# deryrahman/image-caption-emotion-indonesia

Measured on AMD Instinct MI355X. Metric: images/sec (train step) + NLL loss match, batch=64 ResNet152+FactoredLSTM-512, higher is better.
Workload: dtype f32 (trunk: operands as 2 f16 pieces each, 3 MFMA products per multiply, f32 accumulate; decoder: large products as 3 bf16 pieces per operand, 6 MFMA products per multiply, the rest f32 MFMA; the persistent LSTM kernel the trunk's split-f16 scheme)

## Files before the change

### image-caption-emotion-indonesia_amd/csrc/fused_block.hip

```cpp
#include <cstdlib>
#include <type_traits>

#include "common.h"
#include "mfma_core.h"
#include "kernels.h"

namespace capnet {
namespace {

typedef _Float16 h8 __attribute__((ext_vector_type(8)));
typedef _Float16 h4 __attribute__((ext_vector_type(4)));
typedef _Float16 h2 __attribute__((ext_vector_type(2)));
typedef float f2 __attribute__((ext_vector_type(2)));

constexpr int kFHdr = 4;

__host__ __device__ constexpr int fb_kslot(int g, int j) { return 16 * (j >> 2) + 4 * g + (j & 3); }

__device__ __forceinline__ void fb_split4(const f32x4 v, h4& h, h4& l) {
  const f2 a = {v[0], v[1]}, b = {v[2], v[3]};
  const h2 ha = __builtin_convertvector(a, h2), hb = __builtin_convertvector(b, h2);
  const f2 ra = a - __builtin_convertvector(ha, f2), rb = b - __builtin_convertvector(hb, f2);
  const h2 la = __builtin_convertvector(ra, h2), lb = __builtin_convertvector(rb, h2);
  h = h4{ha[0], ha[1], hb[0], hb[1]};
// ... 242 lines not shown
}

constexpr int kQC = 16;

template <int K>
__global__ __launch_bounds__(K * 4) void fb_quad_kernel(const float* __restrict__ G, const float* __restrict__ mu,
                                                        const float* __restrict__ w , int C, double inv_count,
                                                        double unbias, const float* __restrict__ gamma, const float* __restrict__ beta,
                                                        float* __restrict__ running_mean, float* __restrict__ running_var,
                                                        float momentum, float eps, float* __restrict__ scale, float* __restrict__ shift,
                                                        float* __restrict__ batch_mean, float* __restrict__ batch_var, int* __restrict__ err) {
  constexpr int NW = K / 16, S = K / 4, SB = S < 32 ? S : 32;
  __shared__ float red[2][kQC][NW];
  const int tid = threadIdx.x, lane = tid & 63, nb = tid >> 6, g4 = lane >> 4, ln = lane & 15, c0 = blockIdx.x * kQC;
  const float* wq = w + (long)blockIdx.x * K * kQC;
  f32x4 acc = {0.f, 0.f, 0.f, 0.f};
#pragma unroll
  for (int s0 = 0; s0 < S; s0 += SB) {
    float a[SB], b[SB];
#pragma unroll
    for (int i = 0; i < SB; ++i) {
      const int k = 4 * (s0 + i) + g4;
      a[i] = wq[k * kQC + ln];
      b[i] = G[(long)k * K + 16 * nb + ln];
    }
#pragma unroll
    for (int i = 0; i < SB; ++i) acc = __builtin_amdgcn_mfma_f32_16x16x4f32(a[i], b[i], acc, 0, 0, 0);
  }
  const int col = 16 * nb + ln;
  const f32x4 wv = *reinterpret_cast<const f32x4*>(wq + col * kQC + 4 * g4);
  const float m = mu[col];
#pragma unroll
  for (int r = 0; r < 4; ++r) {
    float q = acc[r] * wv[r], sm = m * wv[r];
#pragma unroll
    for (int o = 1; o < 16; o <<= 1) {
      q += __shfl_xor(q, o);
      sm += __shfl_xor(sm, o);
    }
    if (ln == 0) { red[0][4 * g4 + r][nb] = q; red[1][4 * g4 + r][nb] = sm; }
  }
  __syncthreads();
  if (tid < kQC && c0 + tid < C) {
    const int c = c0 + tid;
    double qq = 0.0, ss = 0.0;
#pragma unroll
    for (int v = 0; v < NW; ++v) { qq += (double)red[0][tid][v]; ss += (double)red[1][tid][v]; }
    if (err && !(qq < __builtin_inf())) atomicOr(err, 8);
    const double mean = ss * inv_count;
    double var = qq * inv_count - mean * mean;
    if (var < 0.0) var = 0.0;
    const float invstd = (float)(1.0 / sqrt(var + (double)eps));
    const float gm = gamma ? gamma[c] : 1.f, bt = beta ? beta[c] : 0.f;
    const float sc = gm * invstd;
    scale[c] = sc;
    shift[c] = bt - (float)mean * sc;
    if (running_mean) {
      running_mean[c] = __builtin_fmaf(momentum, (float)mean, (1.f - momentum) * running_mean[c]);
      running_var[c] = __builtin_fmaf(momentum, (float)(var * unbias), (1.f - momentum) * running_var[c]);
    }
    if (batch_mean) {
      batch_mean[c] = (float)mean;
      batch_var[c] = (float)(var * unbias);
    }
  }
}

struct FArgs {
  const float* y2; const float* s2; const float* t2;
  const unsigned* w3; const unsigned* w1;
  const float* s3; const float* t3;
  const float* res; const float* sd; const float* td;
  float* out; float* y1; float* part_sum; float* part_sq;
  int M, e3, e1;
  int* err;
};

#ifndef CAPNET_FB_DBG
#define CAPNET_FB_DBG 0
#endif
template <int N>
__device__ __forceinline__ void fb_wait_vmcnt() { asm volatile("s_waitcnt vmcnt(%0)" ::"n"(N) : "memory"); }

template <int MID, int RS, int NW>
__global__ __launch_bounds__(64 * NW, NW / 4) void fb_fused_kernel(const FArgs g) {
  constexpr int C = 4 * MID, KS = MID / 32, NB = MID / 16, NCH = C / 32;
  constexpr int SLOT = MID * 128;
  constexpr int NDMA = SLOT / 1024 / NW;
  constexpr int L = 2 * RS;
  constexpr int TR = 16 * RS * NW;
  constexpr int NT = 64 * NW;
  static_assert(NDMA >= 1 && 4 * NDMA + 2 * L <= 63, "vmcnt range");
  __shared__ __attribute__((aligned(16))) unsigned char ring[4 * SLOT];
  __shared__ __attribute__((aligned(16))) float par[4][C];
  const int tid = threadIdx.x, lane = tid & 63, wave = tid >> 6, gq = lane >> 4, ln = lane & 15;
  const int wave_u = __builtin_amdgcn_readfirstlane(wave);
  const unsigned ring0 = __builtin_amdgcn_readfirstlane((unsigned)(size_t)(__attribute__((address_space(3))) unsigned char*)ring);
  const int tile0 = (int)blockIdx.x * TR;
  const bool fold_res = g.sd != nullptr;
  const float* const w3img = reinterpret_cast<const float*>(g.w3 + kFHdr);
  const float* const w1img = reinterpret_cast<const float*>(g.w1 + kFHdr);

  auto dma = [&](const float* img, int cc, int slot) __attribute__((always_inline)) {
    const float* src = img + (long)cc * (SLOT / 4);
#pragma unroll
    for (int q = 0; q < ((CAPNET_FB_DBG == 2 || CAPNET_FB_DBG == 4) ? 0 : NDMA); ++q)
      glds16(src, (wave_u * NDMA + q) * 1024 + lane * 16, ring0 + (unsigned)(slot * SLOT + (wave_u * NDMA + q) * 1024));
  };
  unsigned idoff[RS];
#pragma unroll
  for (int s = 0; s < RS; ++s) {
    const int row = min(tile0 + (wave * RS + s) * 16 + ln, g.M - 1);
    idoff[s] = (unsigned)(((long)row * C + 4 * gq) * 4);
  }
  f32x4 idA[RS][2], idB[RS][2];
  auto fetch_id = [&](int cc, f32x4 (&id)[RS][2]) __attribute__((always_inline)) {
#pragma unroll
    for (int s = 0; s < RS; ++s)
#pragma unroll
      for (int blk = 0; blk < 2; ++blk) gload16(id[s][blk], g.res, idoff[s] + (unsigned)((32 * cc + 16 * blk) * 4));
  };

  dma(w3img, 0, 0);
  dma(w1img, 0, 1);
  fetch_id(0, idA);
  fetch_id(NCH > 1 ? 1 : 0, idB);
  {
    const float x3 = ldexpf(1.f, -((int)g.w3[0] + g.e3));
    for (int i = tid; i < C; i += NT) {
      par[0][i] = g.s3[i] * x3;
      par[1][i] = g.t3[i];
      par[2][i] = fold_res ? g.sd[i] : 1.f;
      par[3][i] = fold_res ? g.td[i] : 0.f;
    }
  }
  h8 ah[RS][KS], al[RS][KS];
  {
    const float is3 = ldexpf(1.f, g.e3);
#pragma unroll
    for (int s = 0; s < RS; ++s) {
      const int row = min(tile0 + (wave * RS + s) * 16 + ln, g.M - 1);
      const float* p = g.y2 + (long)row * MID + 4 * gq;
#pragma unroll
      for (int ks = 0; ks < KS; ++ks) {
        f32x4 v0 = *reinterpret_cast<const f32x4*>(p + 32 * ks), v1 = *reinterpret_cast<const f32x4*>(p + 32 * ks + 16);
        const f32x4 sa = *reinterpret_cast<const f32x4*>(g.s2 + 32 * ks + 4 * gq), sb = *reinterpret_cast<const f32x4*>(g.s2 + 32 * ks + 16 + 4 * gq);
        const f32x4 ta = *reinterpret_cast<const f32x4*>(g.t2 + 32 * ks + 4 * gq), tb = *reinterpret_cast<const f32x4*>(g.t2 + 32 * ks + 16 + 4 * gq);
#pragma unroll
        for (int e = 0; e < 4; ++e) {
          v0[e] = fmaxf(fmaf(v0[e], sa[e], ta[e]), 0.f) * is3;
          v1[e] = fmaxf(fmaf(v1[e], sb[e], tb[e]), 0.f) * is3;
        }
        h4 h0, l0, h1, l1;
        fb_split4(v0, h0, l0);
        fb_split4(v1, h1, l1);
        ah[s][ks] = fb_cat(h0, h1);
        al[s][ks] = fb_cat(l0, l1);
      }
    }
  }
  fb_wait_vmcnt<0>();
  CAPNET_LANDED4(idA[0][0], idA[0][1], idB[0][0], idB[0][1]);
  if constexpr (RS == 2) CAPNET_LANDED4(idA[1][0], idA[1][1], idB[1][0], idB[1][1]);
  __syncthreads();

  f32x4 acc[RS][NB];
#pragma unroll
  for (int s = 0; s < RS; ++s)
// ... 74 lines not shown
    for (int bb = 0; bb < FD; ++bb)
      if (bb < NBATB) read_b(bb);
    __builtin_amdgcn_sched_barrier(0);
    fb_wait_vmcnt<4 * NDMA + 2 * L>();
    if constexpr (RS == 2) CAPNET_LANDED4(id[0][0], id[0][1], id[1][0], id[1][1]);
    else CAPNET_LANDED2(id[0][0], id[0][1]);
    h8 oh[RS], ol[RS];
#pragma unroll
    for (int s = 0; s < RS; ++s) {
      const int row = min(tile0 + (wave * RS + s) * 16 + ln, g.M - 1);
      h4 hh[2], ll[2];
#pragma unroll
      for (int blk = 0; blk < 2; ++blk) {
        const int ch = 32 * cc + 16 * blk + 4 * gq;
        const f32x4 sv = *reinterpret_cast<const f32x4*>(&par[0][ch]), tv = *reinterpret_cast<const f32x4*>(&par[1][ch]);
        f32x4 r = id[s][blk], o;
        if (fold_res) {
          const f32x4 dv = *reinterpret_cast<const f32x4*>(&par[2][ch]), ev = *reinterpret_cast<const f32x4*>(&par[3][ch]);
#pragma unroll
          for (int e = 0; e < 4; ++e) r[e] = fmaf(r[e], dv[e], ev[e]);
        }
#pragma unroll
        for (int e = 0; e < 4; ++e) o[e] = fmaxf(fmaf(d[s][blk][e], sv[e], tv[e]) + r[e], 0.f);
        *reinterpret_cast<f32x4*>(g.out + (long)row * C + ch) = o;
        fb_split4(o * is1, hh[blk], ll[blk]);
      }
      oh[s] = fb_cat(hh[0], hh[1]);
      ol[s] = fb_cat(ll[0], ll[1]);
    }
    fetch_id(cc + 2 < NCH ? cc + 2 : NCH - 1, id);
#pragma unroll
    for (int b = 0; b < NBATB; ++b) {
      if (b + FD < NBATB) read_b(b + FD);
      __builtin_amdgcn_sched_barrier(0);
#pragma unroll
      for (int q = 0; q < GB; ++q) {
        const int nb = b * GB + q;
        if (nb < NB) {
#pragma unroll
          for (int s = 0; s < RS; ++s) {
            if (CAPNET_FB_DBG >= 3) continue;
            if (CAPNET_FB_DBG == 1) { asm volatile("" :: "v"(fb[b % (FD + 1)][q][1]), "v"(fb[b % (FD + 1)][q][0])); continue; }
            acc[s][nb] = __builtin_amdgcn_mfma_f32_16x16x32_f16(ol[s], fb[b % (FD + 1)][q][0], acc[s][nb], 0, 0, 0);
            acc[s][nb] = __builtin_amdgcn_mfma_f32_16x16x32_f16(oh[s], fb[b % (FD + 1)][q][1], acc[s][nb], 0, 0, 0);
            acc[s][nb] = __builtin_amdgcn_mfma_f32_16x16x32_f16(oh[s], fb[b % (FD + 1)][q][0], acc[s][nb], 0, 0, 0);
          }
        }
      }
      __builtin_amdgcn_sched_barrier(0);
    }
  };
  auto head = [&](int k) __attribute__((always_inline)) {
    if (k < 4) fb_wait_vmcnt<0>(); else fb_wait_vmcnt<NDMA + 2 * L>();
    __syncthreads();
    const int p = k + 2 < 2 * NCH ? k + 2 : 2 * NCH - 2 + (k & 1);
    dma((p & 1) ? w1img : w3img, p >> 1, (k + 2) & 3);
  };
  static_assert(NCH % 2 == 0, "chunks come in pairs (two named register sets)");
  auto run = [&](auto lag_c) __attribute__((always_inline)) {
    constexpr int LAG = decltype(lag_c)::value;
    for (int k = 0; k < 2 * NCH; k += 4) {
      const int c0 = k >> 1;
      head(k);
      if constexpr (LAG == 0) phase_a(c0);
      else { if (c0 > 0) phase_b(c0 - 1, idB); }
      head(k + 1);
      if constexpr (LAG == 0) phase_b(c0, idA);
      else phase_a(c0);
      head(k + 2);
      if constexpr (LAG == 0) phase_a(c0 + 1);
      else phase_b(c0, idA);
      head(k + 3);
      if constexpr (LAG == 0) phase_b(c0 + 1, idB);
      else phase_a(c0 + 1);
    }
    if constexpr (NW == 8) {
      head(2 * NCH);
      if constexpr (LAG != 0) phase_b(NCH - 1, idB);
    }
    fb_wait_vmcnt<0>();
    CAPNET_LANDED4(idA[0][0], idA[0][1], idB[0][0], idB[0][1]);
    if constexpr (RS == 2) CAPNET_LANDED4(idA[1][0], idA[1][1], idB[1][0], idB[1][1]);
  };
  if (NW == 4 || wave_u < 4) run(std::integral_constant<int, 0>{});
  else run(std::integral_constant<int, 1>{});
  __syncthreads();

  const float osc = ldexpf(1.f, -((int)g.w1[0] + g.e1));
  float (*const scratch)[NW][MID] = reinterpret_cast<float (*)[NW][MID]>(ring);
  float bad = 0.f;
#pragma unroll
  for (int nb = 0; nb < NB; ++nb) {
    float cs = 0.f, cq = 0.f;
#pragma unroll
    for (int s = 0; s < RS; ++s)
#pragma unroll
      for (int i = 0; i < 4; ++i) {
        const int row = tile0 + (wave * RS + s) * 16 + 4 * gq + i;
        const float v = acc[s][nb][i] * osc;
        if (row < g.M) {
          g.y1[(long)row * MID + 16 * nb + ln] = v;
          cs += v;
          cq = fmaf(v, v, cq);
        }
      }
    if (g.part_sum) {
      cs += __shfl_xor(cs, 16); cq += __shfl_xor(cq, 16);
      cs += __shfl_xor(cs, 32); cq += __shfl_xor(cq, 32);
      if (gq == 0) { scratch[0][wave][16 * nb + ln] = cs; scratch[1][wave][16 * nb + ln] = cq; }
    } else {
      bad += cq;
    }
  }
  if (!g.part_sum) {
    if (g.err) flag_nonfinite(bad, g.err);
    return;
  }
  __syncthreads();
  for (int c = tid; c < MID; c += NT) {
    float a = 0.f, b = 0.f;
#pragma unroll
    for (int w = 0; w < NW; ++w) { a += scratch[0][w][c]; b += scratch[1][w][c]; }
    g.part_sum[(long)blockIdx.x * MID + c] = a;
    g.part_sq[(long)blockIdx.x * MID + c] = b;
  }
}

template <int MID>
__global__ __launch_bounds__(256, 1) void fb_fused_wide_kernel(const FArgs g) {
  constexpr int C = 4 * MID, KS = MID / 16, NB = MID / 32, NCH = C / 32, NW = 4;
  constexpr int SLOT = MID * 128;
  constexpr int NDMA = SLOT / 1024 / NW;
  constexpr int L = 4;
  constexpr int TR = 32 * NW;
  constexpr int NT = 64 * NW;
  static_assert(NDMA >= 1 && 4 * NDMA + 2 * L <= 63, "vmcnt range");
  __shared__ __attribute__((aligned(16))) unsigned char ring[4 * SLOT];
  __shared__ __attribute__((aligned(16))) float par[4][C];
  const int tid = threadIdx.x, lane = tid & 63, wave = tid >> 6, lh = lane >> 5, li = lane & 31;
  const int wave_u = __builtin_amdgcn_readfirstlane(wave);
  const unsigned ring0 = __builtin_amdgcn_readfirstlane((unsigned)(size_t)(__attribute__((address_space(3))) unsigned char*)ring);
  const int tile0 = (int)blockIdx.x * TR;
  const bool fold_res = g.sd != nullptr;
  const float* const w3img = reinterpret_cast<const float*>(g.w3 + kFHdr);
  const float* const w1img = reinterpret_cast<const float*>(g.w1 + kFHdr);
  auto dma = [&](const float* img, int cc, int slot) __attribute__((always_inline)) {
    const float* src = img + (long)cc * (SLOT / 4);
#pragma unroll
    for (int q = 0; q < ((CAPNET_FB_DBG == 2 || CAPNET_FB_DBG == 4) ? 0 : NDMA); ++q)
      glds16(src, (wave_u * NDMA + q) * 1024 + lane * 16, ring0 + (unsigned)(slot * SLOT + (wave_u * NDMA + q) * 1024));
  };
  const int myrow = min(tile0 + wave * 32 + li, g.M - 1);
  const unsigned idoff = (unsigned)(((long)myrow * C + 4 * lh) * 4);
  f32x4 idA[4], idB[4];
  auto fetch_id = [&](int cc, f32x4 (&id)[4]) __attribute__((always_inline)) {
#pragma unroll
    for (int q = 0; q < 4; ++q) gload16(id[q], g.res, idoff + (unsigned)((32 * cc + 8 * q) * 4));
  };
  dma(w3img, 0, 0);
  dma(w1img, 0, 1);
  fetch_id(0, idA);
  fetch_id(NCH > 1 ? 1 : 0, idB);
  {
    const float x3 = ldexpf(1.f, -((int)g.w3[0] + g.e3));
    for (int i = tid; i < C; i += NT) {
      par[0][i] = g.s3[i] * x3;
      par[1][i] = g.t3[i];
// ... 179 lines not shown
#pragma unroll
    for (int w = 0; w < NW; ++w) { a += scratch[0][w][c]; b += scratch[1][w][c]; }
    g.part_sum[(long)blockIdx.x * MID + c] = a;
    g.part_sq[(long)blockIdx.x * MID + c] = b;
  }
}

}

bool fused_block_shape_ok(long M, int MID) {
  return (MID == 64 || MID == 128 || MID == 256) && M > 0 && M < (1l << 24) && M * 4 * MID * 4 < (1l << 32);
}

size_t fused_block_weight_words(int C, int MID, int role) {
  return (size_t)kFHdr + (size_t)C * MID * (role == 0 ? 2 : 1);
}

static bool fb_wide(int MID) {
  const char* e = getenv("CAPNET_FB_WIDE");
  if (e && (e[0] == '0' || e[0] == '1')) return e[0] == '1';
  (void)MID;
  return false;
}

int fused_block_pack(const float* w, unsigned* img, int C, int MID, int role, hipStream_t stream) {
  CAPNET_REQUIRE(w && img && aligned16(img) && C == 4 * MID && (MID == 64 || MID == 128 || MID == 256) && (role == 0 || role == 1),
                 "fused_block_pack: bad argument (C=%d MID=%d role=%d)", C, MID, role);
  CAPNET_HIP_CHECK(hipMemsetAsync(img, 0, kFHdr * 4, stream));
  const long n = (long)C * MID;
  hipLaunchKernelGGL(fb_absmax_kernel, dim3((int)(cdiv(n, 256 * 8) > 1024 ? 1024 : cdiv(n, 256 * 8))), dim3(256), 0, stream, w, img, n);
  CAPNET_LAUNCH_CHECK();
  hipLaunchKernelGGL(fb_pack_kernel, dim3((int)(cdiv(n / 4, 256) > 2048 ? 2048 : cdiv(n / 4, 256))), dim3(256), 0, stream, w, img, C, MID, role, fb_wide(MID) ? 1 : 0);
  CAPNET_LAUNCH_CHECK();
  return kOk;
}

int fused_block_gram_slices(long M, int K) { return cdiv(M, fb_gram_rows(K)); }
int fused_block_gram_pairs(int K) { const int nb = K / 64; return nb * (nb + 1) / 2; }
size_t fused_block_stats_floats(long M, int K) {
  const size_t s = fused_block_gram_slices(M, K), p = fused_block_gram_pairs(K);
  return s * p * 4096 + ((s * K + 3) / 4 * 4) + ((size_t)K * K + K) + 8;
}

int fused_block_stats(const float* y2, const float* s2, const float* t2, const unsigned* w3img, long M, int MID, int in_exp,
                      const float* gamma, const float* beta, float* running_mean, float* running_var, float momentum, float eps,
                      float* scale, float* shift, float* batch_mean, float* batch_var, float* work, int* err, hipStream_t stream) {
  CAPNET_REQUIRE(y2 && s2 && t2 && w3img && scale && shift && work && aligned16(work) && aligned16(y2) && fused_block_shape_ok(M, MID) &&
                     in_exp > -64 && in_exp < 64, "fused_block_stats: bad argument");
  const int K = MID, C = 4 * MID;
  GArgs a;
  a.y2 = y2; a.s2 = s2; a.t2 = t2; a.M = (int)M; a.K = K; a.in_exp = in_exp;
  a.slices = fused_block_gram_slices(M, K); a.pairs = fused_block_gram_pairs(K); a.slice_rows = fb_gram_rows(K);
  a.gp = work;
  a.cs = work + (size_t)a.slices * a.pairs * 4096;
  float* G = a.cs + ((size_t)a.slices * K + 3) / 4 * 4;
  float* mu = G + (size_t)K * K;
  if (K == 256) hipLaunchKernelGGL(fb_gram_kernel<256>, dim3(a.slices), dim3(256), 0, stream, a);
  else if (K == 128) hipLaunchKernelGGL(fb_gram_kernel<128>, dim3(a.slices), dim3(256), 0, stream, a);
  else hipLaunchKernelGGL(fb_gram_kernel<64>, dim3(a.slices), dim3(256), 0, stream, a);
  hipLaunchKernelGGL(fb_gram_reduce_kernel, dim3(cdiv((long)K * K + K, 32)), dim3(256), 0, stream, a.gp, a.cs, G, mu, K, a.slices, a.pairs);
  const double inv = 1.0 / (double)M, unbias = M > 1 ? (double)M / (double)(M - 1) : 1.0;
  const float* wcopy = reinterpret_cast<const float*>(w3img + kFHdr + (size_t)C * MID);
  if (K == 256)
    hipLaunchKernelGGL(fb_quad_kernel<256>, dim3(cdiv(C, kQC)), dim3(K * 4), 0, stream, G, mu, wcopy, C, inv, unbias, gamma, beta,
                       running_mean, running_var, momentum, eps, scale, shift, batch_mean, batch_var, err);
  else if (K == 128)
    hipLaunchKernelGGL(fb_quad_kernel<128>, dim3(cdiv(C, kQC)), dim3(K * 4), 0, stream, G, mu, wcopy, C, inv, unbias, gamma, beta,
                       running_mean, running_var, momentum, eps, scale, shift, batch_mean, batch_var, err);
  else
    hipLaunchKernelGGL(fb_quad_kernel<64>, dim3(cdiv(C, kQC)), dim3(K * 4), 0, stream, G, mu, wcopy, C, inv, unbias, gamma, beta,
                       running_mean, running_var, momentum, eps, scale, shift, batch_mean, batch_var, err);
  CAPNET_LAUNCH_CHECK();
  return kOk;
}

static void fb_shape(int MID, int* rs, int* nw) {
  (void)MID;
  const char* e = getenv("CAPNET_FB_RS");
  const char* w = getenv("CAPNET_FB_NW");
  *nw = (w && w[0] == '4') ? 4 : 8;
  *rs = (e && (e[0] == '1' || e[0] == '2')) ? e[0] - '0' : (*nw == 8 ? 1 : 2);
  if (*nw == 8) *rs = 1;
}
int fused_block_tiles(long M, int MID) {
  if (fb_wide(MID)) return cdiv(M, 128);
  int rs, nw;
  fb_shape(MID, &rs, &nw);
  return cdiv(M, 16 * rs * nw);
}

int fused_block_forward(const float* y2, const float* s2, const float* t2, const unsigned* w3img, const float* s3, const float* t3,
                        const float* res, const float* sd, const float* td, float* out, const unsigned* w1img, float* y1,
                        float* part_sum, float* part_sq, long M, int MID, int e3, int e1, int* err, hipStream_t stream) {
  CAPNET_REQUIRE(y2 && s2 && t2 && w3img && s3 && t3 && res && out && w1img && y1 && fused_block_shape_ok(M, MID),
                 "fused_block_forward: bad argument");
  CAPNET_REQUIRE(aligned16(y2) && aligned16(s2) && aligned16(t2) && aligned16(w3img) && aligned16(w1img) && aligned16(res) &&
                     aligned16(out) && (sd == nullptr) == (td == nullptr) && (part_sum == nullptr) == (part_sq == nullptr) &&
                     e3 > -64 && e3 < 64 && e1 > -64 && e1 < 64, "fused_block_forward: alignment / pairs / exponents");
  FArgs a;
  a.y2 = y2; a.s2 = s2; a.t2 = t2; a.w3 = w3img; a.w1 = w1img; a.s3 = s3; a.t3 = t3; a.res = res; a.sd = sd; a.td = td;
  a.out = out; a.y1 = y1; a.part_sum = part_sum; a.part_sq = part_sq; a.M = (int)M; a.e3 = e3; a.e1 = e1; a.err = err;
  const dim3 grid(fused_block_tiles(M, MID));
  int rs, nw;
  fb_shape(MID, &rs, &nw);
  if (fb_wide(MID)) {
    const dim3 block(256);
    if (MID == 256) CAPNET_LAUNCH_TIMED((fb_fused_wide_kernel<256>), grid, block, stream, a);
    else if (MID == 128) CAPNET_LAUNCH_TIMED((fb_fused_wide_kernel<128>), grid, block, stream, a);
    else CAPNET_LAUNCH_TIMED((fb_fused_wide_kernel<64>), grid, block, stream, a);
    CAPNET_LAUNCH_CHECK();
    return kOk;
  }
  const dim3 block(64 * nw);
  if (nw == 8) {
    if (MID == 256) CAPNET_LAUNCH_TIMED((fb_fused_kernel<256, 1, 8>), grid, block, stream, a);
    else if (MID == 128) CAPNET_LAUNCH_TIMED((fb_fused_kernel<128, 1, 8>), grid, block, stream, a);
    else CAPNET_LAUNCH_TIMED((fb_fused_kernel<64, 1, 8>), grid, block, stream, a);
  } else if (rs == 2) {
    if (MID == 256) CAPNET_LAUNCH_TIMED((fb_fused_kernel<256, 2, 4>), grid, block, stream, a);
    else if (MID == 128) CAPNET_LAUNCH_TIMED((fb_fused_kernel<128, 2, 4>), grid, block, stream, a);
    else CAPNET_LAUNCH_TIMED((fb_fused_kernel<64, 2, 4>), grid, block, stream, a);
  } else {
    if (MID == 256) CAPNET_LAUNCH_TIMED((fb_fused_kernel<256, 1, 4>), grid, block, stream, a);
    else if (MID == 128) CAPNET_LAUNCH_TIMED((fb_fused_kernel<128, 1, 4>), grid, block, stream, a);
    else CAPNET_LAUNCH_TIMED((fb_fused_kernel<64, 1, 4>), grid, block, stream, a);
  }
  CAPNET_LAUNCH_CHECK();
  return kOk;
}

}
```

### image-caption-emotion-indonesia_amd/csrc/conv3x3_patch.hip

```cpp
#include <cstdlib>

#include "common.h"
#include "mfma_core.h"
#include "kernels.h"

namespace capnet {
namespace {

typedef _Float16 h8 __attribute__((ext_vector_type(8)));
typedef _Float16 h4 __attribute__((ext_vector_type(4)));
typedef _Float16 h2 __attribute__((ext_vector_type(2)));
typedef float f2 __attribute__((ext_vector_type(2)));
typedef unsigned u4 __attribute__((ext_vector_type(4)));

constexpr int PBM = 128;
constexpr int kPmax = 248;
constexpr int kPatchSub = kPmax * 16;
constexpr int kPatch = 8 * kPatchSub;
constexpr int kThreads = 512;
constexpr int kPL = (kPmax * 8 + kThreads - 1) / kThreads;
constexpr int kHdrWords = 4;
static_assert(kPmax % 16 == 8 && kPmax >= PBM + 2 * 56 + 2, "patch size");

struct PArgs {
  const float* x;
  const unsigned* wimg;
  float* y;
  const float* in_scale;
  const float* in_shift;
  float* part_sum;
  float* part_sq;
  int M, Cin, Cout, relu_in, H, W;
  int in_exp;
  int* err;
  int tiles_m, tiles_n;
  unsigned tn_mul, tn_sh, hw_mul, hw_sh, w_mul, w_sh;
  const float* res;
  const float* res_scale;
  const float* res_shift;
  float* tail_out;
};

__device__ __forceinline__ void p_split4(const f32x4 v, h4& h, h4& l) {
  const f2 a = {v[0], v[1]}, b = {v[2], v[3]};
  const h2 ha = __builtin_convertvector(a, h2), hb = __builtin_convertvector(b, h2);
  const f2 ra = a - __builtin_convertvector(ha, f2), rb = b - __builtin_convertvector(hb, f2);
  const h2 la = __builtin_convertvector(ra, h2), lb = __builtin_convertvector(rb, h2);
  h = h4{ha[0], ha[1], hb[0], hb[1]};
  l = h4{la[0], la[1], lb[0], lb[1]};
}
__device__ __forceinline__ unsigned p_cell(int row, int c) {
  const int r = row & 15;
  return (unsigned)((row * 2 + (c ^ ((r >> 3) & 1))) * 16);
}

template <int BN, int MODE>
__global__ __launch_bounds__(kThreads, MODE == 0 ? 4 : 2) void conv3x3_patch_kernel(const PArgs g) {
  constexpr bool KSPLIT = MODE == 1, WIDE = MODE == 2;
  static_assert(!WIDE || BN == 256, "the wide arrangement is the 256-column tile's");
  constexpr int WN = WIDE ? 4 : 2;
  constexpr int NT = BN / (32 * WN);
  constexpr int MT = MODE == 0 ? 1 : 2;
  constexpr int kSubB = BN * 2 * 16, kImgB = 4 * kSubB;
  constexpr int kRing = 3;
  constexpr int NDMA = kImgB / 1024 / 8;
  static_assert(NDMA * 8 * 1024 == kImgB, "weight image per wave");
  constexpr int kXch = KSPLIT ? 8 * NT * 16 * 64 * 4 : 0;
  constexpr int kLds = kPatch + kRing * kImgB > kXch ? kPatch + kRing * kImgB : kXch;
  __shared__ __attribute__((aligned(16))) unsigned char lds[kLds];
  float (*const scratch)[4][BN] = reinterpret_cast<float (*)[4][BN]>(lds);
  static_assert(2 * 4 * BN * 4 <= kPatch, "statistics scratch inside the patch");
  unsigned char* const patch = lds;
  unsigned char* const bbuf = lds + kPatch;
  const int tid = threadIdx.x, lane = tid & 63, wave = tid >> 6;
  const int kq2 = KSPLIT ? (wave & 1) : 0;
  const int wm = MODE == 0 ? (wave >> 1) : (wave >> 2), wn = KSPLIT ? ((wave >> 1) & 1) : WIDE ? (wave & 3) : (wave & 1);
  const int rows0 = wm * (32 * MT);
  const int li = lane & 31, lh = lane >> 5;
  const int W = g.W, Cin = g.Cin;
  const int nkc = Cin / 32, nk = 9 * nkc;
  const int total = g.tiles_m * g.tiles_n, G = (int)gridDim.x;
  const float oscale = ldexpf(1.f, -((int)g.wimg[0] + g.in_exp));
  const float iscale = ldexpf(1.f, g.in_exp);
  const int pq = tid & 7;
  const unsigned char* const a_rd = patch + (kq2 * 2 + lh) * kPatchSub + (rows0 + li) * 16;
  const unsigned char* const b_rd = bbuf + p_cell(wn * (BN / WN) + li, lh);
  const int wave_u = __builtin_amdgcn_readfirstlane(wave);
  const unsigned lds_b0 = __builtin_amdgcn_readfirstlane((unsigned)(size_t)(__attribute__((address_space(3))) unsigned char*)bbuf);

  for (int wk = (int)blockIdx.x; wk < total; wk += G) {
    const int id = xcd_remap(wk, total);
    const int tm = (int)fast_div((unsigned)id, g.tn_mul, g.tn_sh), tn = id - tm * g.tiles_n;
    const int m0 = tm * PBM, n0 = tn * BN;
    const int pb = m0 - W - 1;
    const int P = PBM + 2 * W + 2;
    unsigned vmask[MT];
#pragma unroll
    for (int mt = 0; mt < MT; ++mt) {
      const int m = m0 + rows0 + mt * 32 + li;
      const int mc = m < g.M ? m : g.M - 1;
      const int b = (int)fast_div((unsigned)mc, g.hw_mul, g.hw_sh), rem = mc - b * g.H * W;
      const int oh = (int)fast_div((unsigned)rem, g.w_mul, g.w_sh), ow = rem - oh * W;
      unsigned vm = 0;
#pragma unroll
      for (int t = 0; t < 9; ++t) {
        const int ih = oh + t / 3 - 1, iw = ow + t % 3 - 1;
        if ((unsigned)ih < (unsigned)g.H && (unsigned)iw < (unsigned)W) vm |= 1u << t;
      }
      vmask[mt] = vm;
    }
    const float* wsrc = reinterpret_cast<const float*>(g.wimg + kHdrWords) + (long)tn * nk * (kImgB / 4);

    f32x4 pre[kPL], fs, ft;
    auto fetch_patch = [&](int c) {
#pragma unroll
      for (int u = 0; u < kPL; ++u) {
        const int px = (tid >> 3) + (kThreads / 8) * u;
        const long p = (long)pb + px;
        f32x4 v = {0.f, 0.f, 0.f, 0.f};
        if (px < P && p >= 0 && p < g.M) v = *reinterpret_cast<const f32x4*>(g.x + p * Cin + c * 32 + 4 * pq);
        pre[u] = v;
      }
      if (g.in_scale) {
        fs = *reinterpret_cast<const f32x4*>(g.in_scale + c * 32 + 4 * pq);
        ft = *reinterpret_cast<const f32x4*>(g.in_shift + c * 32 + 4 * pq);
      }
    };
    auto stage_patch = [&]() {
      unsigned char* d = patch + (pq >> 1) * kPatchSub + (pq & 1) * 8;
      const f32x4 fs2 = fs * iscale, ft2 = ft * iscale;
#pragma unroll
      for (int u = 0; u < kPL; ++u) {
        const int px = (tid >> 3) + (kThreads / 8) * u;
        if (px < P) {
          f32x4 v = pre[u];
          if (g.in_scale) {
#pragma unroll
            for (int e = 0; e < 4; ++e) v[e] = fmaf(v[e], fs2[e], ft2[e]);
          } else {
            v *= iscale;
          }
          if (g.relu_in) {
#pragma unroll
            for (int e = 0; e < 4; ++e) v[e] = fmaxf(v[e], 0.f);
          }
          h4 h, l;
          p_split4(v, h, l);
          *reinterpret_cast<h4*>(d + px * 16) = h;
          *reinterpret_cast<h4*>(d + 4 * kPatchSub + px * 16) = l;
        }
      }
    };
    auto dma_b = [&](int kt, int buf) {
      const float* src = wsrc + (long)kt * (kImgB / 4);
#pragma unroll
      for (int q = 0; q < NDMA; ++q)
        glds16(src, (wave_u * NDMA + q) * 1024 + lane * 16, lds_b0 + (unsigned)(buf * kImgB + (wave_u * NDMA + q) * 1024));
    };

    f32x16 acc[MT][NT];
#pragma unroll
    for (int mt = 0; mt < MT; ++mt)
#pragma unroll
      for (int nt = 0; nt < NT; ++nt)
#pragma unroll
        for (int r = 0; r < 16; ++r) acc[mt][nt][r] = 0.f;

    auto kt_of = [&](int s2) { const int c2 = s2 / 9; return (s2 - 9 * c2) * nkc + c2; };
    fetch_patch(0);
    __syncthreads();
#pragma unroll
    for (int r = 0; r < kRing - 1; ++r)
      if (r < nk) dma_b(kt_of(r), r);
    int step = 0;
    for (int c = 0; c < nkc; ++c) {
      if (c > 0) __syncthreads();
      stage_patch();
      if (c + 1 < nkc) fetch_patch(c + 1);
#pragma unroll
      for (int t = 0; t < 9; ++t, ++step) {
        constexpr int kR = kRing;
        const int buf = t % kR;
        if (step + kRing - 2 < nk) asm volatile("s_waitcnt vmcnt(%0)" ::"n"((kRing - 2) * NDMA) : "memory");
        else asm volatile("s_waitcnt vmcnt(0)" ::: "memory");
        __syncthreads();
        if (step + kRing - 1 < nk) {
          const int s2 = step + kRing - 1, c2 = s2 / 9;
          dma_b((s2 - 9 * c2) * nkc + c2, (t + kR - 1) % kR);
        }
        const int toff = ((t / 3) * W + t % 3) * 16;
#pragma unroll
        for (int gi = 0; gi < (KSPLIT ? 1 : 2); ++gi) {
          const int gsel = KSPLIT ? kq2 : gi;
          h8 af[MT][2], bf[NT][2];
#pragma unroll
          for (int mt = 0; mt < MT; ++mt) {
            const bool ok = (vmask[mt] >> t) & 1u;
#pragma unroll
            for (int p = 0; p < 2; ++p) {
              const h8 v = *reinterpret_cast<const h8*>(a_rd + (p * 4 + gi * 2) * kPatchSub + mt * 512 + toff);
              const h8 z = {0, 0, 0, 0, 0, 0, 0, 0};
              af[mt][p] = ok ? v : z;
            }
          }
#pragma unroll
          for (int nt = 0; nt < NT; ++nt)
#pragma unroll
            for (int p = 0; p < 2; ++p)
              bf[nt][p] = *reinterpret_cast<const h8*>(b_rd + buf * kImgB + (p * 2 + gsel) * kSubB + nt * 1024);
#pragma unroll
          for (int mt = 0; mt < MT; ++mt)
#pragma unroll
            for (int nt = 0; nt < NT; ++nt) {
              acc[mt][nt] = __builtin_amdgcn_mfma_f32_32x32x16_f16(af[mt][1], bf[nt][0], acc[mt][nt], 0, 0, 0);
              acc[mt][nt] = __builtin_amdgcn_mfma_f32_32x32x16_f16(af[mt][0], bf[nt][1], acc[mt][nt], 0, 0, 0);
              acc[mt][nt] = __builtin_amdgcn_mfma_f32_32x32x16_f16(af[mt][0], bf[nt][0], acc[mt][nt], 0, 0, 0);
            }
        }
      }
    }
    if (KSPLIT) {
      __syncthreads();
      float* xch = reinterpret_cast<float*>(lds) + (long)wave * (NT * 16 * 64);
#pragma unroll
      for (int nt = 0; nt < NT; ++nt)
#pragma unroll
        for (int r = 0; r < 16; ++r) xch[(nt * 16 + r) * 64 + lane] = kq2 ? acc[0][nt][r] : acc[MT - 1][nt][r];
      __syncthreads();
    }
    constexpr int NFIN = WIDE ? 2 : 1;
    float cs[NFIN][NT], cq[NFIN][NT];
    {
      const float* xin = reinterpret_cast<const float*>(lds) + (long)(wave ^ 1) * (NT * 16 * 64);
#pragma unroll
      for (int f = 0; f < NFIN; ++f) {
        const int mb = WIDE ? f : kq2;
#pragma unroll
        for (int nt = 0; nt < NT; ++nt) {
          cs[f][nt] = 0.f;
          cq[f][nt] = 0.f;
#pragma unroll
          for (int r = 0; r < 16; ++r) {
            const int row = m0 + rows0 + mb * 32 + 4 * lh + (r & 3) + 8 * (r >> 2);
            float v = WIDE ? acc[f][nt][r] : (kq2 ? acc[MT - 1][nt][r] : acc[0][nt][r]);
            if (KSPLIT) v += xin[(nt * 16 + r) * 64 + lane];
            v *= oscale;
            if (row < g.M) {
              g.y[(long)row * g.Cout + n0 + wn * (BN / WN) + nt * 32 + li] = v;
              cs[f][nt] += v;
              cq[f][nt] = fmaf(v, v, cq[f][nt]);
            }
          }
        }
      }
    }
    if (!g.part_sum && g.err) {
      float t = 0.f;
#pragma unroll
      for (int f = 0; f < NFIN; ++f)
#pragma unroll
        for (int nt = 0; nt < NT; ++nt) t += cq[f][nt];
      flag_nonfinite(t, g.err);
    }
    if (g.part_sum) {
      __syncthreads();
#pragma unroll
      for (int f = 0; f < NFIN; ++f) {
        const int rb = MODE == 0 ? wm : wm * 2 + (WIDE ? f : kq2);
#pragma unroll
        for (int nt = 0; nt < NT; ++nt) {
          cs[f][nt] += __shfl_xor(cs[f][nt], 32);
          cq[f][nt] += __shfl_xor(cq[f][nt], 32);
          if (lh == 0) {
            scratch[0][rb][wn * (BN / WN) + nt * 32 + li] = cs[f][nt];
            scratch[1][rb][wn * (BN / WN) + nt * 32 + li] = cq[f][nt];
          }
        }
      }
      __syncthreads();
      if (tid < BN) {
        g.part_sum[(long)tm * g.Cout + n0 + tid] = (scratch[0][0][tid] + scratch[0][1][tid]) + (scratch[0][2][tid] + scratch[0][3][tid]);
        g.part_sq[(long)tm * g.Cout + n0 + tid] = (scratch[1][0][tid] + scratch[1][1][tid]) + (scratch[1][2][tid] + scratch[1][3][tid]);
      }
    }
  }
}

template <int BN>
__global__ __launch_bounds__(kThreads, BN == 256 ? 2 : 4) void conv1x1_tail_kernel(const PArgs g) {
  constexpr int MT = BN == 256 ? 2 : 1;
  constexpr int WN = BN == 256 ? 4 : 2;
  constexpr int NT = BN / (32 * WN);
  constexpr int kSubB = BN * 2 * 16, kImgB = 4 * kSubB;
  constexpr int kRing = 3;
  constexpr int NDMA = kImgB / 1024 / 8;
  constexpr int kSubA = PBM * 16, kImgA = 8 * kSubA;
  __shared__ __attribute__((aligned(16))) unsigned char lds[2 * kImgA + kRing * kImgB];
  static_assert(2 * (8 / WN) * BN * 4 <= kImgA, "the statistics' scratch lies over an A buffer (see the end of a tile)");
  unsigned char* const abuf = lds;
  unsigned char* const bbuf = lds + 2 * kImgA;
  const int tid = threadIdx.x, lane = tid & 63, wave = tid >> 6;
  const int wm = BN == 256 ? wave >> 2 : wave >> 1, wn = BN == 256 ? (wave & 3) : (wave & 1);
  const int li = lane & 31, lh = lane >> 5;
// ... 265 lines not shown
```

Baseline: 9016.

## Add one-barrier-per-chunk schedule for eight-wave fused bottleneck kernel

Adds a BAR=2 variant of the eight-wave fused bottleneck kernel. In it, all waves run both phases of a chunk back to back, with a single wait and barrier per chunk. The weight DMA for the next chunk is issued right after that barrier. This replaces the lagged two-group schedule, which needs a barrier at every half-step. The new variant is the default for MID 64 and 128 and can be overridden with an environment variable. It gives up the overlap between the two wave groups' phases in exchange for fewer synchronisations.

Result: no change. 9041 (median of 6 runs) (+0.3%).

```diff
diff --git a/image-caption-emotion-indonesia_amd/csrc/fused_block.hip b/image-caption-emotion-indonesia_amd/csrc/fused_block.hip
--- a/image-caption-emotion-indonesia_amd/csrc/fused_block.hip
+++ b/image-caption-emotion-indonesia_amd/csrc/fused_block.hip
@@ -348,8 +348,9 @@
 template <int N>
 __device__ __forceinline__ void fb_wait_vmcnt() { asm volatile("s_waitcnt vmcnt(%0)" ::"n"(N) : "memory"); }
 
-template <int MID, int RS, int NW>
+template <int MID, int RS, int NW, int BAR = 1>
 __global__ __launch_bounds__(64 * NW, NW / 4) void fb_fused_kernel(const FArgs g) {
+  static_assert(BAR == 1 || (BAR == 2 && NW == 8 && RS == 1), "one barrier per chunk: the eight-wave form only");
   constexpr int C = 4 * MID, KS = MID / 32, NB = MID / 16, NCH = C / 32;
   constexpr int SLOT = MID * 128;
   constexpr int NDMA = SLOT / 1024 / NW;
@@ -590,7 +591,27 @@
     CAPNET_LANDED4(idA[0][0], idA[0][1], idB[0][0], idB[0][1]);
     if constexpr (RS == 2) CAPNET_LANDED4(idA[1][0], idA[1][1], idB[1][0], idB[1][1]);
   };
-  if (NW == 4 || wave_u < 4) run(std::integral_constant<int, 0>{});
+  auto head2 = [&](int c) __attribute__((always_inline)) {
+    if (c > 0) fb_wait_vmcnt<2 * L>();
+    __syncthreads();
+    const int n = c + 1 < NCH ? c + 1 : NCH - 1;
+    dma(w3img, n, (2 * c + 2) & 3);
+    dma(w1img, n, (2 * c + 3) & 3);
+  };
+  auto run2 = [&]() __attribute__((always_inline)) {
+    for (int c = 0; c < NCH; c += 2) {
+      head2(c);
+      phase_a(c);
+      phase_b(c, idA);
+      head2(c + 1);
+      phase_a(c + 1);
+      phase_b(c + 1, idB);
+    }
+    fb_wait_vmcnt<0>();
+    CAPNET_LANDED4(idA[0][0], idA[0][1], idB[0][0], idB[0][1]);
+  };
+  if constexpr (BAR == 2) run2();
+  else if (NW == 4 || wave_u < 4) run(std::integral_constant<int, 0>{});
   else run(std::integral_constant<int, 1>{});
   __syncthreads();
 
@@ -936,6 +957,11 @@
   *rs = (e && (e[0] == '1' || e[0] == '2')) ? e[0] - '0' : (*nw == 8 ? 1 : 2);
   if (*nw == 8) *rs = 1;
 }
+static int fb_bar(int MID) {
+  const char* e = getenv("CAPNET_FB_BAR");
+  if (e && (e[0] == '1' || e[0] == '2')) return e[0] - '0';
+  return MID == 256 ? 1 : 2;
+}
 int fused_block_tiles(long M, int MID) {
   if (fb_wide(MID)) return cdiv(M, 128);
   int rs, nw;
@@ -966,7 +992,11 @@
     return kOk;
   }
   const dim3 block(64 * nw);
-  if (nw == 8) {
+  if (nw == 8 && fb_bar(MID) == 2) {
+    if (MID == 256) CAPNET_LAUNCH_TIMED((fb_fused_kernel<256, 1, 8, 2>), grid, block, stream, a);
+    else if (MID == 128) CAPNET_LAUNCH_TIMED((fb_fused_kernel<128, 1, 8, 2>), grid, block, stream, a);
+    else CAPNET_LAUNCH_TIMED((fb_fused_kernel<64, 1, 8, 2>), grid, block, stream, a);
+  } else if (nw == 8) {
     if (MID == 256) CAPNET_LAUNCH_TIMED((fb_fused_kernel<256, 1, 8>), grid, block, stream, a);
     else if (MID == 128) CAPNET_LAUNCH_TIMED((fb_fused_kernel<128, 1, 8>), grid, block, stream, a);
     else CAPNET_LAUNCH_TIMED((fb_fused_kernel<64, 1, 8>), grid, block, stream, a);
```

## Issue patch loads asynchronously mid-tap and fold them into the ring's vmcnt schedule

Applied to the files above, without the earlier changes.

The next channel chunk's input patch loads are now issued as raw buffer loads with clamped addresses at tap 6, not right after staging. Out-of-range rows are zeroed at staging time instead. The per-tap waitcnt values are retuned so the patch loads and the three-deep weight DMA ring share one vmcnt budget, which keeps the global loads in flight across several MFMA taps. Debug switches under a compile-time flag, off by default, can disable the DMA, the fragment loads or the MFMAs for profiling. The hand-counted waits are fragile and depend on the exact number of loads issued.

Result: no change. 8645 before, 8638 after (median of 6 runs) (-0.1%).

```diff
diff --git a/image-caption-emotion-indonesia_amd/csrc/conv3x3_patch.hip b/image-caption-emotion-indonesia_amd/csrc/conv3x3_patch.hip
--- a/image-caption-emotion-indonesia_amd/csrc/conv3x3_patch.hip
+++ b/image-caption-emotion-indonesia_amd/csrc/conv3x3_patch.hip
@@ -21,6 +21,10 @@
 constexpr int kPL = (kPmax * 8 + kThreads - 1) / kThreads;
 constexpr int kHdrWords = 4;
 static_assert(kPmax % 16 == 8 && kPmax >= PBM + 2 * 56 + 2, "patch size");
+#ifndef CAPNET_P3_DBG
+#define CAPNET_P3_DBG 0
+#endif
+constexpr int kDbg = CAPNET_P3_DBG;
 
 struct PArgs {
   const float* x;
@@ -48,6 +52,10 @@
   const h2 la = __builtin_convertvector(ra, h2), lb = __builtin_convertvector(rb, h2);
   h = h4{ha[0], ha[1], hb[0], hb[1]};
   l = h4{la[0], la[1], lb[0], lb[1]};
+}
+__device__ __forceinline__ h8 dbg_frag(int v) {
+  const _Float16 f = (_Float16)(float)(v & 7);
+  return h8{f, f, f, f, f, f, f, f};
 }
 __device__ __forceinline__ unsigned p_cell(int row, int c) {
   const int r = row & 15;
@@ -111,20 +119,23 @@
     }
     const float* wsrc = reinterpret_cast<const float*>(g.wimg + kHdrWords) + (long)tn * nk * (kImgB / 4);
 
+    constexpr int nP = kPL + 2;
+    static_assert(kPL == 4, "CAPNET_LANDED4 below lands the four patch loads");
     f32x4 pre[kPL], fs, ft;
+    const int pb0 = pb > 0 ? pb : 0;
+    const float* const ps_base = g.in_scale ? g.in_scale : reinterpret_cast<const float*>(g.wimg);
+    const float* const pt_base = g.in_shift ? g.in_shift : reinterpret_cast<const float*>(g.wimg);
     auto fetch_patch = [&](int c) {
+      const float* src = g.x + (long)pb0 * Cin + c * 32;
 #pragma unroll
       for (int u = 0; u < kPL; ++u) {
         const int px = (tid >> 3) + (kThreads / 8) * u;
-        const long p = (long)pb + px;
-        f32x4 v = {0.f, 0.f, 0.f, 0.f};
-        if (px < P && p >= 0 && p < g.M) v = *reinterpret_cast<const f32x4*>(g.x + p * Cin + c * 32 + 4 * pq);
-        pre[u] = v;
-      }
-      if (g.in_scale) {
-        fs = *reinterpret_cast<const f32x4*>(g.in_scale + c * 32 + 4 * pq);
-        ft = *reinterpret_cast<const f32x4*>(g.in_shift + c * 32 + 4 * pq);
-      }
+        int p = pb + px;
+        p = p < 0 ? 0 : p < g.M ? p : g.M - 1;
+        gload16(pre[u], src, (unsigned)((p - pb0) * Cin + 4 * pq) * 4u);
+      }
+      gload16(fs, ps_base + c * 32, 16u * pq);
+      gload16(ft, pt_base + c * 32, 16u * pq);
     };
     auto stage_patch = [&]() {
       unsigned char* d = patch + (pq >> 1) * kPatchSub + (pq & 1) * 8;
@@ -133,7 +144,9 @@
       for (int u = 0; u < kPL; ++u) {
         const int px = (tid >> 3) + (kThreads / 8) * u;
         if (px < P) {
-          f32x4 v = pre[u];
+          const int p = pb + px;
+          const f32x4 z = {0.f, 0.f, 0.f, 0.f};
+          f32x4 v = p >= 0 && p < g.M ? pre[u] : z;
           if (g.in_scale) {
 #pragma unroll
             for (int e = 0; e < 4; ++e) v[e] = fmaf(v[e], fs2[e], ft2[e]);
@@ -152,6 +165,7 @@
       }
     };
     auto dma_b = [&](int kt, int buf) {
+      if (kDbg & 4) return;
       const float* src = wsrc + (long)kt * (kImgB / 4);
 #pragma unroll
       for (int q = 0; q < NDMA; ++q)
@@ -172,22 +186,31 @@
 #pragma unroll
     for (int r = 0; r < kRing - 1; ++r)
       if (r < nk) dma_b(kt_of(r), r);
+    constexpr int kTP = 6;
+    static_assert(kRing == 3 && kTP + 2 < 9, "wait counts below assume a three-deep ring, patch fetched at tap 6");
     int step = 0;
     for (int c = 0; c < nkc; ++c) {
       if (c > 0) __syncthreads();
+      if (kDbg & 4) asm volatile("s_waitcnt vmcnt(0)" ::: "memory");
+      else asm volatile("s_waitcnt vmcnt(%0)" ::"n"(2 * NDMA) : "memory");
+      CAPNET_LANDED4(pre[0], pre[1], pre[2], pre[3]);
+      CAPNET_LANDED2(fs, ft);
       stage_patch();
-      if (c + 1 < nkc) fetch_patch(c + 1);
+      const bool more = c + 1 < nkc;
 #pragma unroll
       for (int t = 0; t < 9; ++t, ++step) {
         constexpr int kR = kRing;
         const int buf = t % kR;
-        if (step + kRing - 2 < nk) asm volatile("s_waitcnt vmcnt(%0)" ::"n"((kRing - 2) * NDMA) : "memory");
-        else asm volatile("s_waitcnt vmcnt(0)" ::: "memory");
-        __syncthreads();
+        if (kDbg & 4) {
+        } else if (t <= kTP) asm volatile("s_waitcnt vmcnt(%0)" ::"n"(NDMA) : "memory");
+        else if (t == kTP + 1 || more) asm volatile("s_waitcnt vmcnt(%0)" ::"n"(NDMA + nP) : "memory");
+        else asm volatile("s_waitcnt vmcnt(%0)" ::"n"(nP) : "memory");
+        if (!(kDbg & 8) || t == 0) __syncthreads();
         if (step + kRing - 1 < nk) {
           const int s2 = step + kRing - 1, c2 = s2 / 9;
           dma_b((s2 - 9 * c2) * nkc + c2, (t + kR - 1) % kR);
         }
+        if (t == kTP) fetch_patch(more ? c + 1 : c);
         const int toff = ((t / 3) * W + t % 3) * 16;
 #pragma unroll
         for (int gi = 0; gi < (KSPLIT ? 1 : 2); ++gi) {
@@ -198,8 +221,12 @@
             const bool ok = (vmask[mt] >> t) & 1u;
 #pragma unroll
             for (int p = 0; p < 2; ++p) {
+              const h8 z = {0, 0, 0, 0, 0, 0, 0, 0};
+              if (kDbg & 2) {
+                af[mt][p] = dbg_frag(lane + p);
+                continue;
+              }
               const h8 v = *reinterpret_cast<const h8*>(a_rd + (p * 4 + gi * 2) * kPatchSub + mt * 512 + toff);
-              const h8 z = {0, 0, 0, 0, 0, 0, 0, 0};
               af[mt][p] = ok ? v : z;
             }
           }
@@ -207,7 +234,18 @@
           for (int nt = 0; nt < NT; ++nt)
 #pragma unroll
             for (int p = 0; p < 2; ++p)
-              bf[nt][p] = *reinterpret_cast<const h8*>(b_rd + buf * kImgB + (p * 2 + gsel) * kSubB + nt * 1024);
+              bf[nt][p] = (kDbg & 2) ? dbg_frag(lane + 2 * p + 1)
+                                     : *reinterpret_cast<const h8*>(b_rd + buf * kImgB + (p * 2 + gsel) * kSubB + nt * 1024);
+          if (kDbg & 1) {
+#pragma unroll
+            for (int p = 0; p < 2; ++p) {
+#pragma unroll
+              for (int mt = 0; mt < MT; ++mt) asm volatile("" ::"v"(af[mt][p]));
+#pragma unroll
+              for (int nt = 0; nt < NT; ++nt) asm volatile("" ::"v"(bf[nt][p]));
+            }
+            continue;
+          }
 #pragma unroll
           for (int mt = 0; mt < MT; ++mt)
 #pragma unroll
@@ -219,6 +257,9 @@
         }
       }
     }
+    asm volatile("s_waitcnt vmcnt(0)" ::: "memory");
+    CAPNET_LANDED4(pre[0], pre[1], pre[2], pre[3]);
+    CAPNET_LANDED2(fs, ft);
     if (KSPLIT) {
       __syncthreads();
       float* xch = reinterpret_cast<float*>(lds) + (long)wave * (NT * 16 * 64);
```
